# ucsdarclab/Python-SuPer

Measured on AMD Instinct MI355X. Metric: LM iterations/s (embedded-deformation LM, point-to-plane + ARAP + Rot), higher is better.
Workload: dtype f64; 1 GPU; C2: 200000 surfels / 2000 ED nodes / KNN=4, point-to-plane + ARAP + Rot, 10 LM iterations + Surfels.update per frame; frames_per_gpu=8, streams_per_gpu=1, global_frames=8, parallelism=frames sharded over 1 GPU(s), beta all-gather

## Files before the change

python-super_amd/csrc/slm_api.hip:

```cpp
#include <atomic>
#include <condition_variable>
#include <functional>
#include <mutex>
#include <new>
#include <string>
#include <thread>
#include <algorithm>
#include <vector>
#include <cstdio>
#include <cstring>

#include "slm_common.h"
#include "slm_corr.h"
#include "slm_host.h"
#include "slm_launch.h"
#include "slm_prep.h"

static thread_local std::string g_err;
static const char* const kBadKnn =
    "slm_bind_frame: a KNN index (sf_knn_idx or ed_knn_idx) lies outside [0, J) or a surfel's row of sf_knn_idx repeats an id";

void slm_set_error_text(const char* msg) { g_err = msg; }

namespace {
// ... 163 lines not shown

namespace {
class BindPool {
 public:
  ~BindPool() { shutdown(); }
  void run(int n, const std::function<void(int)>& job) {
    ensure(n - 1);
    {
      std::lock_guard<std::mutex> lk(m_);
      job_ = &job;
      n_active_ = n - 1;
      pending_ = n - 1;
      ++generation_;
    }
    cv_work_.notify_all();
    job(0);
    std::unique_lock<std::mutex> lk(m_);
    cv_done_.wait(lk, [&] { return pending_ == 0; });
    job_ = nullptr;
  }
  void shutdown() {
    {
      std::lock_guard<std::mutex> lk(m_);
      stop_ = true;
    }
    cv_work_.notify_all();
    for (std::thread& t : threads_)
      if (t.joinable()) t.join();
    threads_.clear();
  }

 private:
  void ensure(int n_workers) {
    while ((int)threads_.size() < n_workers) {
      const int id = (int)threads_.size();
      threads_.emplace_back([this, id] { loop(id); });
    }
  }
  void loop(int id) {
    int seen = 0;
    for (;;) {
      const std::function<void(int)>* job = nullptr;
      {
        std::unique_lock<std::mutex> lk(m_);
        cv_work_.wait(lk, [&] { return stop_ || generation_ != seen; });
        if (stop_) return;
        seen = generation_;
        if (id < n_active_) job = job_;
      }
      if (job) {
        (*job)(id + 1);
        std::lock_guard<std::mutex> lk(m_);
        if (--pending_ == 0) cv_done_.notify_all();
      }
    }
  }
  std::vector<std::thread> threads_;
  std::mutex m_;
  std::condition_variable cv_work_, cv_done_;
  const std::function<void(int)>* job_ = nullptr;
  int generation_ = 0, n_active_ = 0, pending_ = 0;
  bool stop_ = false;
};
}

struct slm_solver {
  PrepBuffers* prep = nullptr;
  BindPool bind_pool;
  AsyncWorker prep_worker;
  PrepBuffers* prep_async = nullptr;
  hipStream_t prep_stream = nullptr;
  std::vector<PrepBuffers*> bind_prep;
  std::vector<hipStream_t> bind_streams;
  std::vector<hipEvent_t> bind_events;
  std::mutex band_mutex;
  hipEvent_t drain_event = nullptr;
  double drain_est_ms = 0.0;
  int last_solver_form = -1;
  int last_dag_mode = -1;
  bool no_reuse = false;
  bool hybrid_batches = true;
  long dag_max_nodes = 8000;
  bool fuse_begin = true;
  bool pure_fill = true;
  bool profile = false;
  std::vector<hipEvent_t> ev_pool;
  std::vector<std::vector<hipEvent_t>> ev_runs;
  slm_config cfg{};
  std::vector<Slot> slots;
  FrameDev* frames_dev = nullptr;
  int* bw_dev = nullptr;
  int* bw_host = nullptr;
  int* reuse_dev = nullptr;
  int rank = 0, world = 1;
  int corr_mode = 0;
  double corr_w = 0.0;
  CorrDev* corr_dev = nullptr;
  bool shard_mode = false;
};
namespace {
bool solve_is_task_graph(const slm_solver* s, int n, int J);
}

static std::atomic<long long> g_reallocs{0}, g_realloc_bytes{0}, g_plan_builds{0}, g_plan_reuses{0}, g_plan_fill_hits{0};

template <typename T>
static hipError_t grow(T*& p, size_t& cap, size_t need) {
  if (need <= cap) return hipSuccess;
  const size_t want = need + need / 8;
  ++g_reallocs;
  g_realloc_bytes += (long long)(want * sizeof(T));
  return grow(p, cap, need, want);
}
template <typename T>
static hipError_t grow(GP<T>& p, size_t& cap, size_t need) {
  T* q = p;
  const hipError_t e = grow(q, cap, need);
  p = q;
  return e;
}

static int check_slots(slm_solver* s, int first, int n);

extern "C" {

const char* slm_last_error(void) { return g_err.c_str(); }

int slm_debug_last_solver_form(slm_solver* s) { return s ? s->last_solver_form : -1; }
int slm_debug_last_dag_mode(slm_solver* s) { return s ? s->last_dag_mode : -1; }

int slm_debug_counters(int64_t out[4]) {
  if (!out) return fail(SLM_ERR_INVALID, "slm_debug_counters: null output");
  out[0] = g_reallocs;
  out[1] = g_realloc_bytes;
  out[2] = g_plan_builds;
  out[3] = g_plan_reuses;
  return SLM_OK;
}

int slm_debug_dag_timeout(int64_t ticks) {
  if (ticks < 0) return fail(SLM_ERR_INVALID, "slm_debug_dag_timeout: negative");
  HIPCHK(set_dag_timeout_ticks(ticks == 0 ? 300000000ll : (long long)ticks));
  return SLM_OK;
}

int slm_debug_dag_abort(slm_solver* s, int32_t n_frames, void* stream) {
  int rc = check_slots(s, 0, n_frames);
  if (rc) return rc;
  for (int i = 0; i < n_frames; ++i)
    if (!s->slots[i].h.nd_ready) return fail(SLM_ERR_UNSUPPORTED, "slm_debug_dag_abort: every slot needs a nested-dissection plan");
  hipStream_t st = (hipStream_t)stream;
  launch_dag_abort_check(s->frames_dev, n_frames, st);
  launch_accept(s->frames_dev, n_frames, s->cfg.phase_test, 0, std::max(s->cfg.num_iterations, 1), st);
  HIPCHK(hipGetLastError());
  return SLM_OK;
}

int slm_debug_dag_trace(slm_solver* s, int32_t slot, int32_t on, void* stream) {
  if (!s || slot < 0 || slot >= (int)s->slots.size()) return fail(SLM_ERR_INVALID, "slm_debug_dag_trace: bad argument");
  Slot& sl = s->slots[slot];
  if (!sl.h.bound || !sl.h.nd_ready) return fail(SLM_ERR_UNBOUND, "slm_debug_dag_trace: no nested-dissection plan bound");
  hipStream_t st = (hipStream_t)stream;
  if (on) {
    HIPCHK(grow(sl.d_dag_trace, sl.cap_dag_trace, (size_t)24 * sl.h.n_dag_tasks + 8));
    HIPCHK(hipMemsetAsync(sl.d_dag_trace, 0, sizeof(long long) * 24 * (size_t)sl.h.n_dag_tasks, st));
  }
// ... 46 lines not shown
    case 4: src = h.blk_key.get(); n = sizeof(int32_t) * (size_t)h.n_blocks; break;
    case 5: src = h.blk_start.get(); n = sizeof(int32_t) * ((size_t)h.n_blocks + 1); break;
    case 6: src = h.blk_entry.get(); n = sizeof(int32_t) * 10 * (size_t)h.n_runs; break;
    case 7: src = h.v2_ready ? h.wg_first.get() : nullptr; n = h.v2_ready ? sizeof(int32_t) * n_wg : 0; break;
    case 8: src = h.v2_ready ? h.wg_last.get() : nullptr; n = h.v2_ready ? sizeof(int32_t) * n_wg : 0; break;
    case 9: src = h.v2_ready ? h.run_lidx.get() : nullptr; n = h.v2_ready ? 10 * (size_t)h.n_runs : 0; break;
    case 10: src = h.v2_ready ? h.blk2_start.get() : nullptr; n = h.v2_ready ? sizeof(int32_t) * ((size_t)h.n_blocks + 1) : 0; break;
    case 11: src = h.v2_ready ? h.blk2_entry.get() : nullptr; n = h.v2_ready ? sizeof(int32_t) * (size_t)h.n_wblk : 0; break;
    case 12: src = h.s_pts.get(); n = esz * 3 * (size_t)h.n_pos; break;
    default: return fail(SLM_ERR_INVALID, "slm_debug_read_plan: unknown array");
  }
  *n_bytes = (int64_t)n;
  const size_t m = n < (size_t)(max_bytes > 0 ? max_bytes : 0) ? n : (size_t)(max_bytes > 0 ? max_bytes : 0);
  if (m > 0 && host_out && src) HIPCHK(hipMemcpyAsync(host_out, src, m, hipMemcpyDeviceToHost, (hipStream_t)stream));
  HIPCHK(hipStreamSynchronize((hipStream_t)stream));
  return SLM_OK;
}

int slm_abi_version(void) { return SLM_ABI_VERSION; }

int slm_abi_check(int32_t abi_version, int32_t sz_config, int32_t sz_frame, int32_t sz_gf_config, int32_t sz_gf_frame,
                  int32_t sz_iter_record) {
  if (abi_version != SLM_ABI_VERSION || sz_config != (int32_t)sizeof(slm_config) || sz_frame != (int32_t)sizeof(slm_frame) ||
      sz_gf_config != (int32_t)sizeof(slm_gf_config) || sz_gf_frame != (int32_t)sizeof(slm_gf_frame) ||
      sz_iter_record != (int32_t)sizeof(slm_iter_record)) {
    char buf[320];
    snprintf(buf, sizeof(buf),
             "slm_abi_check: caller built for ABI %d (slm_config %d, slm_frame %d, slm_gf_config %d, slm_gf_frame %d, "
             "slm_iter_record %d bytes), library is ABI %d (%zu, %zu, %zu, %zu, %zu)",
             abi_version, sz_config, sz_frame, sz_gf_config, sz_gf_frame, sz_iter_record, SLM_ABI_VERSION, sizeof(slm_config),
             sizeof(slm_frame), sizeof(slm_gf_config), sizeof(slm_gf_frame), sizeof(slm_iter_record));
    return fail(SLM_ERR_INVALID, buf);
  }
  return SLM_OK;
}

int slm_device_count(void) {
  int n = 0;
  if (hipGetDeviceCount(&n) != hipSuccess) return 0;
  return n;
}

int slm_create(const slm_config* cfg, slm_solver** out) {
  if (!cfg || !out) return fail(SLM_ERR_INVALID, "slm_create: null argument");
  if (cfg->max_frames < 1 || cfg->num_iterations < 0 || !(cfg->v > 0.0))
    return fail(SLM_ERR_INVALID, "slm_create: bad config");
  if (cfg->solver_path < 0 || cfg->solver_path > 4) return fail(SLM_ERR_INVALID, "slm_create: solver_path must be 0..4");
  if (cfg->data_path < 0 || cfg->data_path > 2) return fail(SLM_ERR_INVALID, "slm_create: data_path must be 0..2");
  if (slm_device_count() < 1) return fail(SLM_ERR_NO_DEVICE, "slm_create: no HIP device visible");
  slm_solver* s = new (std::nothrow) slm_solver();
  if (!s) return fail(SLM_ERR_HIP, "slm_create: out of host memory");
  s->cfg = *cfg;
  try {
    s->slots.resize(cfg->max_frames);
  } catch (...) {
    delete s;
    return fail(SLM_ERR_HIP, "slm_create: out of host memory");
  }
  hipError_t e = hipMalloc((void**)&s->frames_dev, sizeof(FrameDev) * cfg->max_frames);
  if (e == hipSuccess) e = hipMemset(s->frames_dev, 0, sizeof(FrameDev) * cfg->max_frames);
  if (e == hipSuccess) e = hipMalloc((void**)&s->bw_dev, 2 * sizeof(int));
  if (e == hipSuccess) e = hipMalloc((void**)&s->reuse_dev, sizeof(int) * cfg->max_frames);
  if (e == hipSuccess) e = hipMemset(s->reuse_dev, 0, sizeof(int) * cfg->max_frames);
  if (e == hipSuccess) e = hipHostMalloc((void**)&s->bw_host, 2 * sizeof(int), hipHostMallocDefault);
  if (e == hipSuccess) {
    s->prep = prep_create();
    if (!s->prep) e = hipErrorOutOfMemory;
  }
  if (e != hipSuccess) {
    g_err = std::string("slm_create: ") + hipGetErrorString(e);
    slm_destroy(s);
    return SLM_ERR_HIP;
  }
  {
    int dev = 0;
    (void)hipGetDevice(&dev);
    (void)dag_device_setup(dev, nullptr);
  }
  if (const char* hb = getenv("SLM_HYBRID")) s->hybrid_batches = atoi(hb) != 0;
  if (const char* dm = getenv("SLM_DAG_MAX_NODES")) s->dag_max_nodes = atol(dm);
  if (const char* nr = getenv("SLM_NO_REUSE")) s->no_reuse = atoi(nr) != 0;
  if (const char* pf = getenv("SLM_PURE_FILL")) s->pure_fill = atoi(pf) != 0;
  if (const char* fb = getenv("SLM_FUSE_BEGIN")) s->fuse_begin = atoi(fb) != 0;
  *out = s;
  return SLM_OK;
}

int slm_destroy(slm_solver* s) {
  if (!s) return SLM_OK;
  s->prep_worker.shutdown();
  s->bind_pool.shutdown();
  for (Slot& sl : s->slots) {
    FrameDev& h = sl.h;
    if (h.beta) (void)hipFree(h.beta);
    if (h.delta) (void)hipFree(h.delta);
    if (h.rhs) (void)hipFree(h.rhs);
    if (sl.band) (void)hipFree(sl.band);
    if (sl.linv) (void)hipFree(sl.linv);
    if (h.loss_part) (void)hipFree(h.loss_part);
    if (h.st) (void)hipFree(h.st);
    if (h.rec) (void)hipFree(h.rec);
    if (h.node_pk) (void)hipFree(h.node_pk);
    if (h.tgt_pn) (void)hipFree(h.tgt_pn);
    if (h.tgt_px) (void)hipFree(h.tgt_px);
    if (h.ev_rc) (void)hipFree(h.ev_rc);
    plan_free(sl.plan);
    pairplan_free(sl.pplan);
    if (sl.h_pin) (void)hipHostFree(sl.h_pin);
    sl.h_pairs.release();
    sl.h_knn.release();
    sl.h_pts.release();
    sl.h_pts64.release();
    if (sl.d_fronts) (void)hipFree(sl.d_fronts);
    if (sl.d_items) (void)hipFree(sl.d_items);
    if (sl.d_tile_kind) (void)hipFree(sl.d_tile_kind);
    if (sl.d_zero_tiles) (void)hipFree(sl.d_zero_tiles);
    if (sl.d_ints) (void)hipFree(sl.d_ints);
    if (sl.d_dests) (void)hipFree(sl.d_dests);
    if (sl.d_cur_dests) (void)hipFree(sl.d_cur_dests);
    if (sl.ftiles) (void)hipFree(sl.ftiles);
    if (sl.fvec) (void)hipFree(sl.fvec);
    if (sl.flinv) (void)hipFree(sl.flinv);
    if (sl.fmail) (void)hipFree(sl.fmail);
    if (sl.pairbuf) (void)hipFree(sl.pairbuf);
    if (sl.corr.o) (void)hipFree(sl.corr.o);
    if (sl.corr.n) (void)hipFree(sl.corr.n);
    if (sl.corr.valid) (void)hipFree(sl.corr.valid);
    if (sl.d_dag_flags) (void)hipFree(sl.d_dag_flags);
    if (sl.d_dag_trace) (void)hipFree(sl.d_dag_trace);
    if (sl.prep_fork) (void)hipEventDestroy(sl.prep_fork);
    if (sl.prep_done) (void)hipEventDestroy(sl.prep_done);
  }
  prep_destroy(s->prep);
  prep_destroy(s->prep_async);
  if (s->prep_stream) (void)hipStreamDestroy(s->prep_stream);
  for (PrepBuffers* pb : s->bind_prep) prep_destroy(pb);
  for (hipStream_t q : s->bind_streams) (void)hipStreamDestroy(q);
  for (hipEvent_t e : s->bind_events) (void)hipEventDestroy(e);
  for (auto& evs : s->ev_runs)
    for (hipEvent_t e : evs)
      if (e) (void)hipEventDestroy(e);
  for (hipEvent_t e : s->ev_pool) (void)hipEventDestroy(e);
  if (s->drain_event) (void)hipEventDestroy(s->drain_event);
  if (s->frames_dev) (void)hipFree(s->frames_dev);
  if (s->bw_dev) (void)hipFree(s->bw_dev);
  if (s->reuse_dev) (void)hipFree(s->reuse_dev);
  if (s->corr_dev) (void)hipFree(s->corr_dev);
  if (s->bw_host) (void)hipHostFree(s->bw_host);
  delete s;
  return SLM_OK;
}

static int ensure_band(slm_solver* s, int slot, hipStream_t st) {
  Slot& sl = s->slots[slot];
  if (sl.band_ready) return SLM_OK;
  FrameDev& h = sl.h;
  launch_bandwidth(h.f, s->bw_dev, st);
  HIPCHK(hipMemcpyAsync(s->bw_host, s->bw_dev, 2 * sizeof(int), hipMemcpyDeviceToHost, st));
  HIPCHK(hipStreamSynchronize(st));
  if (s->bw_host[1]) return fail(SLM_ERR_INVALID, kBadKnn);
  int wb = *s->bw_host;
  if (wb > h.nt - 1) wb = h.nt - 1;
  h.wb = wb;
  HIPCHK(grow(sl.band, sl.cap_band, (size_t)h.nt * (wb + 1) * SLM_NB * SLM_NB));
  HIPCHK(grow(sl.linv, sl.cap_linv, (size_t)h.nt * SLM_NB * SLM_NB));
  h.band = sl.band;
// ... 669 lines not shown
  d.fused_begin = d.nd && tuple && d.gram_variants == 1 && d.max_pos > 0 && s->fuse_begin;
  if (tuple && c.phase_test) d.accept_reuse = s->reuse_dev + first;
  d.accept_eval = tuple ? 1 : 0;
  if (d.nd) {
    for (int i = first; i < first + n; ++i) {
      const auto& sc = s->slots[i].cache.nd.sched;
      if (sc.size() > d.sched.size()) d.sched.resize(sc.size(), NDLevelSched{0, 0, 0, 0, 0, -2, 0, -2, 0, -2});
      for (size_t l = 0; l < sc.size(); ++l) {
        NDLevelSched& m = d.sched[l];
        if (m.first == -2) m.first = sc[l].first;
        else if (m.first != sc[l].first || m.n_fronts != sc[l].n_fronts) m.first = -1;
        m.n_fronts = std::max(m.n_fronts, sc[l].n_fronts);
        m.max_npt = std::max(m.max_npt, sc[l].max_npt);
        m.max_nt = std::max(m.max_nt, sc[l].max_nt);
        m.max_pairs = std::max(m.max_pairs, sc[l].max_pairs);
        m.max_n2p = std::max(m.max_n2p, sc[l].max_n2p);
        if (m.schur_at == -2) m.schur_at = sc[l].schur_at;
        else if (m.schur_at != sc[l].schur_at || m.n_schur != sc[l].n_schur) m.schur_at = -1;
        m.n_schur = std::max(m.n_schur, sc[l].n_schur);
        if (m.pull_at == -2) m.pull_at = sc[l].pull_at;
        else if (m.pull_at != sc[l].pull_at || m.n_pull != sc[l].n_pull) m.pull_at = -1;
        m.n_pull = std::max(m.n_pull, sc[l].n_pull);
      }
    }
  }
  if (d.nd && n > 1) {
    for (int i = first; i < first + n; ++i)
      for (size_t l = s->slots[i].cache.nd.sched.size(); l < d.sched.size(); ++l)
        d.sched[l].first = d.sched[l].schur_at = d.sched[l].pull_at = -1;
  }
  for (auto& m : d.sched) {
    if (m.first == -2) m.first = -1;
    if (m.first < 0) m.schur_at = m.pull_at = -1;
    if (m.schur_at == -2) m.schur_at = -1;
    if (m.pull_at == -2) m.pull_at = -1;
  }
  if (s->cfg.use_arap || s->cfg.use_rot)
    d.n_reg_part = std::min(kRegBlocksMax, (d.maxJKe + 255) / 256);
  d.n_acc_part = d.n_reg_part + (s->corr_mode ? kCorrBlocks : 0);
  return d;
}

static bool solve_is_task_graph(const slm_solver* s, int n, int J) {
  return s->cfg.solver_path == 2 || (s->cfg.solver_path == 0 && (n <= 2 || (long)n * J <= s->dag_max_nodes));
}
static bool solve_is_hybrid(const slm_solver* s, int n, const BatchDims& d) {
  return !solve_is_task_graph(s, n, d.maxP / 7) && (s->cfg.solver_path == 4 || (s->cfg.solver_path == 0 && s->hybrid_batches)) &&
         d.hybrid_cut >= 0 && d.hybrid_levels == (int)d.sched.size() && d.hybrid_cut + 1 < d.hybrid_levels;
}
static int dag_cut_of(const slm_solver* s, int n, const BatchDims& d) {
  if (solve_is_task_graph(s, n, d.maxP / 7)) return -1;
  return solve_is_hybrid(s, n, d) ? d.hybrid_cut : -2;
}
int enqueue_front_solve(slm_solver* s, const FrameDev* fr, int n, const BatchDims& d, double u_override, hipStream_t st,
                        bool dag_reset_done = false, bool dag_check_later = false) {
  const bool dag = solve_is_task_graph(s, n, d.maxP / 7);
  const bool hybrid = solve_is_hybrid(s, n, d);
  s->last_solver_form = dag ? 1 : (hybrid ? 2 : 0);
  int mode = -1;
  if (dag) {
    mode = launch_front_solve_dag(fr, n, d.max_tasks, u_override, st, -1, !dag_reset_done, !dag_check_later);
  } else if (hybrid) {
    const int n_levels = (int)d.sched.size(), l_cut = n_levels - 1 - d.hybrid_cut;
    launch_front_levels(fr, n, d.sched.data(), n_levels, l_cut, 0, u_override, st);
    mode = launch_front_solve_dag(fr, n, d.max_top_tasks, u_override, st, d.hybrid_cut, !dag_reset_done, !dag_check_later);
  } else {
    launch_front_solve(fr, n, d.sched.data(), (int)d.sched.size(), u_override, st);
  }
  s->last_dag_mode = mode;
  return mode;
}

void enqueue_zero(const FrameDev* fr, int n, const BatchDims& d, hipStream_t st, const int* reuse, int dag_cut, bool fused) {
  if (!d.nd) launch_iter_begin(fr, n, st);
  else if (!fused) launch_iter_begin_nd(fr, n, st, reuse, dag_cut);
}

void enqueue_jacobian(slm_solver* s, const FrameDev* fr, int n, const BatchDims& d, hipStream_t st, int eval_mode,
                      const int* reuse, int dag_cut, bool fused) {
  const double w = s->cfg.w_data;
  switch (d.form) {
    case DataForm::tuple:
      if (eval_mode >= 0) launch_data_eval(fr, n, kLossBlocks, w, eval_mode, st, reuse);
      if (fused) launch_begin_and_gram(fr, n, d.max_pos, w, st, reuse, dag_cut);
      else launch_data_gram(fr, n, d.max_pos, w, d.gram_variants, st, reuse);
      break;
    case DataForm::pairs:
      launch_data_grad_pairs(fr, n, d.maxN, d.K, w, st);
      if (d.corr) launch_corr_grad_pairs(fr, s->corr_dev + (fr - s->frames_dev), n, d.maxN, d.K, s->corr_mode, s->corr_w, st);
      break;
    case DataForm::per_entry:
      launch_data_grad(fr, n, d.maxN, d.K, w, st);
      if (d.corr) launch_corr_grad(fr, s->corr_dev + (fr - s->frames_dev), n, d.maxN, d.K, s->corr_mode, s->corr_w, st);
      break;
    case DataForm::none: break;
  }
}

enum class Shard { whole, before_exchange, after_exchange };
void enqueue_scatter(slm_solver* s, const FrameDev* fr, int n, const BatchDims& d, hipStream_t st, Shard part) {
  const slm_config& c = s->cfg;
  const bool tuple = d.form == DataForm::tuple;
  if (part == Shard::before_exchange) {
    if (tuple) launch_pair_reduce(fr, n, d.max_blocks, st);
    return;
  }
  if (part == Shard::after_exchange || d.form == DataForm::pairs) launch_pair_scatter(fr, n, d.max_blocks, st);
  else if (tuple && d.nd) launch_front_assemble(fr, n, d.max_blocks, st);
  else if (tuple) launch_band_assemble(fr, n, d.max_blocks, st);
  if (d.nd) {
    launch_reg_grad_nd(fr, n, d.maxP / 7, c.use_arap, c.w_arap, c.use_rot, c.w_rot, st);
    if (!c.use_arap && !c.use_rot) launch_front_load_rhs(fr, n, d.maxP, st);
  } else {
    launch_reg_grad(fr, n, d.maxJKe, c.use_arap, c.w_arap, c.use_rot, c.w_rot, st);
  }
}

void enqueue_data_loss(slm_solver* s, const FrameDev* fr, int n, const BatchDims& d, hipStream_t st, bool at_beta) {
  if (d.form == DataForm::tuple && !at_beta) launch_data_eval(fr, n, kLossBlocks, s->cfg.w_data, 0, st);
  else if (d.form != DataForm::none) launch_data_loss(fr, n, kLossBlocks, d.K, s->cfg.w_data, at_beta ? 0 : 1, st);
  if (s->corr_mode && d.K >= 1)
    launch_corr_loss(fr, s->corr_dev + (fr - s->frames_dev), n, d.K, s->corr_mode, s->corr_w, at_beta ? 0 : 1, 2 * d.n_reg_part,
                     kCorrCntPart, st);
}
}

extern "C" {

static hipEvent_t take_event(slm_solver* s) {
  if (!s->ev_pool.empty()) {
    hipEvent_t e = s->ev_pool.back();
    s->ev_pool.pop_back();
    return e;
  }
  hipEvent_t e = nullptr;
  if (hipEventCreate(&e) != hipSuccess) return nullptr;
  return e;
}

int slm_set_shard(slm_solver* s, int32_t rank, int32_t world) {
  if (!s || world < 1 || rank < 0 || rank >= world) return fail(SLM_ERR_INVALID, "slm_set_shard: bad rank/world");
  if (s->cfg.data_path != 0 || s->cfg.solver_path == 1)
    return fail(SLM_ERR_UNSUPPORTED, "slm_set_shard: needs data_path 0 and a nested-dissection solver_path (0, 2, 3 or 4)");
  if (s->corr_mode)
    return fail(SLM_ERR_UNSUPPORTED, "slm_set_shard: the correspondence term is enabled (slm_enable_corr); it needs every surfel of "
                                     "the frame on one device");
  s->rank = rank;
  s->world = world;
  s->shard_mode = true;
  for (size_t i = 0; i < s->slots.size(); ++i) {
    join_prepare(s, (int)i);
    s->slots[i].model_ready = false;
    s->slots[i].h.bound = 0;
  }
  HIPCHK(hipMemset(s->frames_dev, 0, sizeof(FrameDev) * s->slots.size()));
  return SLM_OK;
}

static int shard_dims(slm_solver* s, int n_frames, BatchDims& d) {
  int rc = check_slots(s, 0, n_frames);
  if (rc) return rc;
  d = dims_of(s, 0, n_frames);
  if (!d.nd || (d.form != DataForm::tuple && d.form != DataForm::pairs))
    return fail(SLM_ERR_UNSUPPORTED, "sharded LM step: every slot needs a multifrontal data path (tuple-sorted or K-generic) and the ND solver");
  return SLM_OK;
}

int slm_lm_grad_local(slm_solver* s, int32_t n_frames, void* stream) {
// ... 582 lines not shown
```

python-super_amd/csrc/slm_begin.h:

```cpp
#pragma once
#include "slm_tile.h"

typedef double dvec2_t __attribute__((ext_vector_type(2)));
__device__ __forceinline__ void zero_pieces(double* base, size_t n_pieces, size_t first, size_t step) {
  const dvec2_t zz = {0.0, 0.0};
  dvec2_t* b2 = reinterpret_cast<dvec2_t*>(base);
  for (size_t pc = first; pc < n_pieces; pc += step) {
    dvec2_t* q = b2 + pc * 1024 + threadIdx.x;
#pragma unroll
    for (int k = 0; k < 4; ++k) __builtin_nontemporal_store(zz, q + 256 * k);
  }
}
__device__ __forceinline__ size_t front_piv_tiles(const NDFront& f) {
  return (size_t)f.npt * f.nt - (size_t)f.npt * (f.npt - 1) / 2;
}
__device__ __forceinline__ void zero_fronts(const FrameDev& fd, int b, int nb) {
  const dvec2_t zz = {0.0, 0.0};
  const int n = fd.n_zero_tiles;
  for (int pc = b; pc < 2 * n; pc += nb) {
    dvec2_t* q = reinterpret_cast<dvec2_t*>(fd.ftiles.get() + fd.zero_tiles[pc >> 1]) + (size_t)(pc & 1) * 1024 + threadIdx.x;
#pragma unroll
    for (int k = 0; k < 4; ++k) __builtin_nontemporal_store(zz, q + 256 * k);
  }
}
__device__ __forceinline__ void iter_begin_nd_body(const FrameDev& fd, int b, int nb, bool reused, int dag_cut, bool gram_sets_count) {
  if (!fd.bound) return;
  if (dag_cut >= -1 && fd.nd_ready && fd.dag_flags) {
    for (int i = b * blockDim.x + threadIdx.x; i < fd.dag_n_flags; i += nb * blockDim.x) fd.dag_flags[i] = 0;
    typedef __attribute__((address_space(1))) long long gll;
    gll* mail = (gll*)(double*)fd.fmail;
    for (int fi = b; fi < fd.n_fronts; fi += nb) {
      const NDFront& f = fd.fronts[fi];
      if (dag_cut >= 0 && f.depth > dag_cut) continue;
      const size_t base = (size_t)(f.linv_off / TILE) * SLM_MAIL_DOUBLES, n = (size_t)f.npt * SLM_MAIL_DOUBLES;
      for (size_t e = threadIdx.x; e < n; e += blockDim.x) mail[base + e] = SLM_MAIL_EMPTY;
    }
  }
  if (fd.st->stopped) return;
  const size_t tid = (size_t)b * blockDim.x + threadIdx.x, nthr = (size_t)nb * blockDim.x;
  const double2 z = make_double2(0.0, 0.0);
  if (fd.nd_ready) {
    zero_fronts(fd, b, nb);
    double2* v2 = reinterpret_cast<double2*>(fd.fvec.get());
    const size_t nv2 = (size_t)fd.zero_vec_doubles / 2;
    for (size_t e = tid; e < nv2; e += nthr) v2[e] = z;
  }
  const size_t nrhs = (size_t)fd.nt * SLM_NB;
  for (size_t e = tid; e < nrhs; e += nthr) fd.rhs[e] = 0.0;
  if (b == 0 && threadIdx.x == 0) {
    if (!reused) {
      if (!gram_sets_count) fd.st->m_grad = 0;
    } else if (fd.pairbuf) {
      fd.st->m_grad = fd.st->m_grad_local;
    }
    fd.st->chol_fail = 0;
  }
}
```

python-super_amd/csrc/slm_data_k4.hip:

```cpp
#include <cstdlib>

#include "slm_data.h"
#include "slm_begin.h"
#include "slm_launch.h"

#define ROW_STRIDE 17

__global__ void __launch_bounds__(256) k_data_eval(const FrameDev* __restrict__ frames, double lam, int mode,
                                                    const int* __restrict__ reuse) {
  __shared__ double sm[16];
  __shared__ int s_skip;
  if (mode == 1 && reuse && reuse[blockIdx.y]) return;
  const FrameDev& fd = frames[blockIdx.y];
  if (!fd.bound || !fd.v1_ready || fd.st->stopped) return;
  if (mode == 1) {
    if (threadIdx.x == 0) s_skip = __hip_atomic_load(&fd.st->eval_valid, __ATOMIC_RELAXED, __HIP_MEMORY_SCOPE_AGENT) == 1;
    __syncthreads();
    if (s_skip) return;
  }
  const double* npk = mode == 0 ? fd.node_pk_try.get() : fd.node_pk.get();
  const int p0 = 256 * fd.wg_lo, p1 = min(fd.n_pos, 256 * fd.wg_hi);
  double acc = 0.0;
  int cnt = 0;
  for (int pos = p0 + blockIdx.x * blockDim.x + threadIdx.x; pos < p1; pos += gridDim.x * blockDim.x) {
    const int4 ids = *reinterpret_cast<const int4*>(fd.s_idx + 4 * (size_t)pos);
    double2 o0 = make_double2(0.0, 0.0), o1 = make_double2(0.0, 0.0);
    if (ids.x >= 0) {
      double wk[4];
      ld_state4(fd.s_w, (size_t)pos, fd.f.state_f64, wk);
      const d3 pp = ld_state3(fd.s_pts, (size_t)pos, fd.f.state_f64);
      SurfelEval ev;
      eval_surfel_core<2, true>(fd, pp, ids, wk, lam, npk, ev);
      if (ev.match) {
        acc += ev.r * ev.r;
        ++cnt;
        o0 = make_double2(ev.r, ev.c[0]);
        o1 = make_double2(ev.c[1], ev.c[2]);
      }
    }
    double2* out = reinterpret_cast<double2*>(fd.ev_rc.get() + 4 * (size_t)pos);
    out[0] = o0;
    out[1] = o1;
  }
  const double s = block_sum(acc, sm);
  const double c = block_sum((double)cnt, sm);
  if (threadIdx.x == 0) {
    fd.loss_part[2 * blockIdx.x] = s;
    fd.loss_part[2 * blockIdx.x + 1] = c;
    LMState* st = fd.st;
    const unsigned long long old = __hip_atomic_fetch_add(&st->eval_acc, (1ull << 32) | (unsigned long long)(unsigned)(int)c,
                                                          __ATOMIC_RELAXED, __HIP_MEMORY_SCOPE_AGENT);
    if ((int)(old >> 32) == (int)gridDim.x - 1) {
      st->m_eval = (int)(unsigned)(old & 0xFFFFFFFFull) + (int)c;
      __hip_atomic_store(&st->eval_acc, 0ull, __ATOMIC_RELAXED, __HIP_MEMORY_SCOPE_AGENT);
      if (mode != 0) __hip_atomic_store(&st->eval_valid, 1, __ATOMIC_RELAXED, __HIP_MEMORY_SCOPE_AGENT);
    }
  }
}

template <bool MERGE, bool BEGIN = false>
__global__ void __launch_bounds__(256, 2) k_data_gram(const FrameDev* __restrict__ frames, double lam,
                                                       int dbg, const int* __restrict__ reuse, int n_gram = 0, int n_begin = 0,
                                                       int dag_cut = -2) {
  if (BEGIN && (int)blockIdx.x >= n_gram) {
    iter_begin_nd_body(frames[blockIdx.y], (int)blockIdx.x - n_gram, n_begin, reuse && reuse[blockIdx.y], dag_cut,
                       frames[blockIdx.y].v1_ready && frames[blockIdx.y].v2_ready);
    return;
  }
  __shared__ double rows[4][64 * ROW_STRIDE];
  __shared__ double recs[MERGE ? SLM_LB_MAX * SLM_WREC : 1];
  __shared__ uint8_t lidx[4][MERGE ? 160 : 4];
  if (reuse && reuse[blockIdx.y]) return;
  const FrameDev& fd = frames[blockIdx.y];
  if (!fd.bound || !fd.v1_ready) return;
  if (MERGE != (fd.v2_ready != 0)) return;
  const int w = threadIdx.x >> 6, l = threadIdx.x & 63;
  const int base = (blockIdx.x * 4 + w) * 64;
  if (blockIdx.x * 256 >= fd.n_pos) return;
  if (blockIdx.x == 0 && threadIdx.x == 0) fd.st->m_grad = fd.st->m_eval;
  if ((int)blockIdx.x < fd.wg_lo || (int)blockIdx.x >= fd.wg_hi) return;
  const bool wact = base < fd.n_pos;
  const int pos = base + l;
  const int lc = l & 15, lq = l >> 4;
  int rec0 = 0, nrec = 0;
  if (MERGE) {
    rec0 = fd.wg_first[blockIdx.x];
    nrec = fd.wg_last[blockIdx.x] - rec0 + 1;
  }
  int my_run = -1;
  int4 ids = {-1, -1, -1, -1};
  double wk[4] = {0, 0, 0, 0};
  d3 pp = {0, 0, 0};
  double2 e0 = make_double2(0.0, 0.0), e1 = make_double2(0.0, 0.0);
  if (wact) {
    my_run = fd.grp_run[(base >> 2) + lc];
    const double2* e2 = reinterpret_cast<const double2*>(fd.ev_rc.get() + 4 * (size_t)pos);
    e0 = e2[0];
    e1 = e2[1];
    ids = *reinterpret_cast<const int4*>(fd.s_idx + 4 * (size_t)pos);
    ld_state4(fd.s_w, (size_t)pos, fd.f.state_f64, wk);
    pp = ld_state3(fd.s_pts, (size_t)pos, fd.f.state_f64);
  }
  uint8_t lv0 = 0, lv1 = 0, lv2 = 0;
  if (MERGE && wact) {
#pragma unroll
    for (int k = 0; k < 3; ++k) {
      const int idx = l + 64 * k;
      const int g = idx / 10, e = idx - 10 * g;
      const int run = __shfl(my_run, g < 16 ? g : 0, 64);
      const uint8_t v = (idx < 160 && run >= 0) ? fd.run_lidx[10 * (size_t)run + e] : (uint8_t)0;
      if (k == 0) lv0 = v; else if (k == 1) lv1 = v; else lv2 = v;
    }
  }
  if (MERGE)
    for (int i = threadIdx.x; i < nrec * SLM_WREC; i += 256) recs[i] = 0.0;
  double* myrow = &rows[w][l * ROW_STRIDE];

  SurfelEval ev;
  ev.match = false;
  ev.r = 0.0;
  ev.id[0] = ev.id[1] = ev.id[2] = ev.id[3] = -1;
  const bool live = wact && ids.x >= 0;
#ifdef SLM_STAMPS
  if (live && !(dbg & 4))
#else
  if (live)
#endif
  {
    ev.id[0] = ids.x; ev.id[1] = ids.y; ev.id[2] = ids.z; ev.id[3] = ids.w;
    ev.match = e0.x != 0.0 || e0.y != 0.0 || e1.x != 0.0 || e1.y != 0.0;
    ev.r = e0.x;
    if (ev.match) rows_from_c(pp, ev.id, wk, lam, fd.node_pk, {e0.y, e1.x, e1.y}, ev.row);
  }
  if (MERGE && wact) {
    lidx[w][l] = lv0;
    lidx[w][l + 64] = lv1;
    if (l + 128 < 160) lidx[w][l + 128] = lv2;
  }
  if (MERGE) __syncthreads();
  if (wact) {

  int slot[4];
#pragma unroll
  for (int k = 0; k < 4; ++k) {
    slot[k] = 0;
#pragma unroll
    for (int k2 = 0; k2 < 4; ++k2) slot[k] += (ev.id[k2] < ev.id[k]) ? 1 : 0;
  }
  double a0[16];
#pragma unroll
  for (int half = 0; half < 2; ++half) {
#pragma unroll
    for (int e = 0; e < 16; ++e) myrow[e] = 0.0;
    if (ev.match) {
#pragma unroll
      for (int k = 0; k < 4; ++k)
#pragma unroll
        for (int c = 0; c < 7; ++c) {
          const int e = 7 * slot[k] + c - 16 * half;
          if (e >= 0 && e < 16) myrow[e] = ev.row[7 * k + c];
        }
      if (half == 1) myrow[28 - 16] = ev.r;
    }
    __builtin_amdgcn_fence(__ATOMIC_RELEASE, "wavefront");
    __builtin_amdgcn_wave_barrier();
    __builtin_amdgcn_fence(__ATOMIC_ACQUIRE, "wavefront");
    if (half == 0) {
#pragma unroll
      for (int g = 0; g < 16; ++g) a0[g] = rows[w][(4 * g + lq) * ROW_STRIDE + lc];
      __builtin_amdgcn_fence(__ATOMIC_RELEASE, "wavefront");
      __builtin_amdgcn_wave_barrier();
      __builtin_amdgcn_fence(__ATOMIC_ACQUIRE, "wavefront");
    }
  }

  double4_t g00 = {0, 0, 0, 0}, g10 = {0, 0, 0, 0}, g11 = {0, 0, 0, 0};
  int cur = -1;

  auto flush = [&](int run, int grp) {
#ifdef SLM_STAMPS
    if (dbg & 1) return;
#endif
    if (MERGE) {
      const uint8_t* lvp = &lidx[w][10 * grp];
#pragma unroll
      for (int t = 0; t < 3; ++t)
#pragma unroll
        for (int r = 0; r < 4; ++r) {
          const int i = 4 * r + lq + (t >= 1 ? 16 : 0), j = lc + (t == 2 ? 16 : 0);
          const double v = t == 0 ? g00[r] : (t == 1 ? g10[r] : g11[r]);
          const int pa = (i * 37) >> 8, pb = (j * 37) >> 8;
          const int ca = i - 7 * pa, cb = j - 7 * pb;
          const bool jrow = (i == 28);
          const bool act = j < 28 && (jrow || (i < 28 && i >= j));
          int ps = jrow ? (pb * (pb + 1) / 2 + pb) : (pa * (pa + 1) / 2 + pb);
          ps = act ? ps : 0;
          const int rec = lvp[ps];
          if (act) unsafeAtomicAdd(&recs[rec * SLM_WREC + (jrow ? 49 + cb : 7 * ca + cb)], v);
        }
    } else {
      double* out = fd.slab + (size_t)run * SLM_SLAB_STRIDE;
#pragma unroll
      for (int r = 0; r < 4; ++r) {
        out[r * 64 + l] = g00[r];
        out[256 + r * 64 + l] = g10[r];
        out[512 + r * 64 + l] = g11[r];
      }
    }
  };

#pragma unroll
  for (int g = 0; g < 16; ++g) {
    const int run = __builtin_amdgcn_readlane(my_run, g);
    if (run != cur) {
      if (cur >= 0) flush(cur, g - 1);
      g00 = double4_t{0, 0, 0, 0};
      g10 = double4_t{0, 0, 0, 0};
      g11 = double4_t{0, 0, 0, 0};
      cur = run;
    }
    if (run < 0) continue;
    const double a1 = rows[w][(4 * g + lq) * ROW_STRIDE + lc];
#ifdef SLM_STAMPS
    if (dbg & 2) { g00[0] += a0[g]; g11[0] += a1; continue; }
#endif
    g00 = __builtin_amdgcn_mfma_f64_16x16x4f64(a0[g], a0[g], g00, 0, 0, 0);
    g10 = __builtin_amdgcn_mfma_f64_16x16x4f64(a1, a0[g], g10, 0, 0, 0);
    g11 = __builtin_amdgcn_mfma_f64_16x16x4f64(a1, a1, g11, 0, 0, 0);
  }
  if (cur >= 0) flush(cur, 15);
  }
  if (MERGE) {
    __syncthreads();
    double* out = fd.wgslab + (size_t)rec0 * SLM_WREC;
    for (int i = threadIdx.x; i < nrec * SLM_WREC; i += 256) out[i] = recs[i];
  }
}

__device__ __forceinline__ double gram_at(const double* g, int i, int j) {
  if (i < 16) return g[16 * i + j];
  if (j < 16) return g[256 + 16 * (i - 16) + j];
  return g[512 + 16 * (i - 16) + (j - 16)];
}

__global__ void __launch_bounds__(256) k_band_assemble(const FrameDev* __restrict__ frames) {
  const FrameDev& fd = frames[blockIdx.y];
  if (!fd.bound || !fd.v1_ready || fd.st->stopped) return;
  const int bi = blockIdx.x * 4 + (threadIdx.x >> 6);
  if (bi >= fd.n_blocks) return;
  const int l = threadIdx.x & 63;
  const unsigned key = (unsigned)fd.blk_key[bi];
  const int a = (int)(key / (unsigned)fd.f.J), b = (int)(key % (unsigned)fd.f.J);
  const int ca = l / 7, cb = l % 7;
  const bool act = (l < 49) && (a != b || ca >= cb);
  const bool jt = (a == b) && l >= 49 && l < 56;
  double acc = 0.0;
  if (fd.v2_ready) {
    const int s0 = fd.blk2_start[bi], s1 = fd.blk2_start[bi + 1];
    if (l < SLM_WREC)
      for (int s = s0; s < s1; ++s) acc += fd.wgslab[(size_t)fd.blk2_entry[s] * SLM_WREC + l];
  } else {
    const int s0 = fd.blk_start[bi], s1 = fd.blk_start[bi + 1];
    for (int s = s0; s < s1; ++s) {
      const int pl = fd.blk_entry[s];
      const int run = pl >> 4, pa = (pl >> 2) & 3, pb = pl & 3;
      const double* G = fd.slab + (size_t)run * SLM_SLAB_STRIDE;
      if (act) acc += gram_at(G, 7 * pa + ca, 7 * pb + cb);
      else if (jt) acc += gram_at(G, 28, 7 * pa + (l - 49));
    }
  }
  if (act) *band_entry(fd, 7 * a + ca, 7 * b + cb) = acc;
  else if (jt) fd.rhs[7 * a + (l - 49)] = -acc;
}

void launch_begin_and_gram(const FrameDev* frames_dev, int n_frames, int max_pos, double lam, hipStream_t st, const int* reuse,
                           int dag_cut) {
  int dbg = 0;
#ifdef SLM_STAMPS
  if (const char* e = getenv("SLM_DBG")) dbg = atoi(e);
#endif
  const int n_gram = (max_pos + 255) / 256, n_begin = 1024;
  hipLaunchKernelGGL((k_data_gram<true, true>), dim3(n_gram + n_begin, n_frames), dim3(256), 0, st, frames_dev, lam, dbg, reuse, n_gram,
                     n_begin, dag_cut);
}

void launch_data_gram(const FrameDev* frames_dev, int n_frames, int max_pos, double lam, int variants,
                      hipStream_t st, const int* reuse) {
  if (max_pos <= 0) return;
  int dbg = 0;
#ifdef SLM_STAMPS
  if (const char* e = getenv("SLM_DBG")) dbg = atoi(e);
#endif
  const dim3 grid((max_pos + 255) / 256, n_frames);
  if (variants & 1) hipLaunchKernelGGL(k_data_gram<true>, grid, dim3(256), 0, st, frames_dev, lam, dbg, reuse);
  if (variants & 2) hipLaunchKernelGGL(k_data_gram<false>, grid, dim3(256), 0, st, frames_dev, lam, dbg, reuse);
}

void launch_data_eval(const FrameDev* frames_dev, int n_frames, int n_blocks, double lam, int mode, hipStream_t st,
                      const int* reuse) {
  hipLaunchKernelGGL(k_data_eval, dim3(n_blocks, n_frames), dim3(256), 0, st, frames_dev, lam, mode, reuse);
}

void launch_band_assemble(const FrameDev* frames_dev, int n_frames, int max_blocks, hipStream_t st) {
  if (max_blocks <= 0) return;
  hipLaunchKernelGGL(k_band_assemble, dim3((max_blocks + 3) / 4, n_frames), dim3(256), 0, st, frames_dev);
}
```

python-super_amd/csrc/slm_launch.h:

```cpp
#pragma once
#include "slm_common.h"

void launch_data_grad(const FrameDev*, int, int, int, double, hipStream_t);
void launch_data_grad_pairs(const FrameDev*, int, int, int, double, hipStream_t);
void launch_data_loss(const FrameDev*, int, int, int, double, int, hipStream_t);
void launch_data_resid(const FrameDev*, int, int, int, double, double*, uint8_t*, int32_t*, hipStream_t);

void launch_data_gram(const FrameDev*, int, int, double, int, hipStream_t, const int* reuse = nullptr);
void launch_begin_and_gram(const FrameDev*, int, int, double, hipStream_t, const int* reuse, int dag_cut);
void launch_data_eval(const FrameDev*, int, int, double, int mode, hipStream_t, const int* reuse = nullptr);
void launch_band_assemble(const FrameDev*, int, int, hipStream_t);

void launch_front_assemble(const FrameDev*, int, int, hipStream_t);
void launch_pair_reduce(const FrameDev*, int, int, hipStream_t);
void launch_pair_scatter(const FrameDev*, int, int, hipStream_t);
void launch_reg_grad_nd(const FrameDev*, int, int, int, double, int, double, hipStream_t);
void launch_front_load_rhs(const FrameDev*, int, int, hipStream_t);
void launch_iter_begin_nd(const FrameDev*, int, hipStream_t, const int* reuse, int dag_cut);
void launch_front_solve(const FrameDev*, int, const NDLevelSched*, int, double, hipStream_t);
void launch_front_levels(const FrameDev*, int, const NDLevelSched*, int, int, int, double, hipStream_t);

bool ensure_dynamic_lds(const void* kernel, size_t bytes);

int launch_front_solve_dag(const FrameDev*, int, int, double, hipStream_t, int cut, bool reset, bool check);
int dag_device_setup(int dev, int* xcd8_out);
int dag_last_mode();
hipError_t set_dag_timeout_ticks(long long);
void launch_dag_abort_check(const FrameDev*, int, hipStream_t);

void launch_bandwidth(const slm_frame&, int*, hipStream_t);
void launch_band_solve(const FrameDev*, int, int, int, double, hipStream_t);
void launch_band_to_dense(const FrameDev*, int, double*, hipStream_t);
void launch_dense_to_band(const FrameDev*, const double*, const double*, hipStream_t);

void launch_reg_grad(const FrameDev*, int, int, int, double, int, double, hipStream_t);
void launch_after_solve(const FrameDev*, int, int, int, int, double, int, double, int, hipStream_t);
void launch_reg_loss(const FrameDev*, int, int, int, double, int, double, int, hipStream_t);

void launch_init_slot(const FrameDev*, int, int, const slm_config&, hipStream_t);
void launch_iter_begin(const FrameDev*, int, hipStream_t);
void launch_pack_nodes(const FrameDev*, int, int, hipStream_t);
void launch_make_trial(const FrameDev*, int, int, hipStream_t);
void launch_pack_target(int, const float*, const float*, float4*, hipStream_t);
void launch_pack_target_px(int, const int*, const uint8_t*, const float*, const float*, float4*, hipStream_t);
void launch_accept(const FrameDev*, int, int, int, int, hipStream_t, int* reuse = nullptr, int eval_pass = 0);
void launch_loss_out(const FrameDev*, int, int, double*, hipStream_t);
void launch_zero_reg_part(const FrameDev*, int, int, hipStream_t);
void launch_update(int, int, int, float*, float*, const int*, const float*, float*, float*, const double*, hipStream_t);
void launch_update64(int, int, int, double*, double*, const int*, const double*, double*, double*, const double*,
                     hipStream_t);
void launch_knn(int, int, int, int, const float*, const float*, int*, float*, hipStream_t);
void launch_knn64(int, int, int, int, const double*, const double*, const int*, const int*, int*, double*, int*,
                  hipStream_t);
void launch_knn_weights64(int, int, int, const int*, const double*, const double*, int, const double*, const double*,
                          double*, uint8_t*, hipStream_t);
void launch_knn_weights(int, int, int, const int*, const float*, const float*, float*, uint8_t*, hipStream_t);
```

Before: 3335 LM it/s.

## Make data Gram kernel persistent with prefetch and interleaved front zeroing

Turns the k_data_gram kernel into a persistent grid sized from the CU count (2*CUs/frames by default, overridable by SLM_GRAM_WGS). Each workgroup loops over a contiguous range of 256-surfel chunks and software-prefetches the next chunk's inputs and lidx while computing the current one. In the fused begin variant, the front-tile zeroing that used to run in separate extra blocks is now spread across the same workgroups and interleaved with the chunk loop. The aim is to cut launch and tail overhead and to hide load latency behind MFMA work, at the cost of extra register pressure from the double-buffered chunk state and the risk of load imbalance across workgroups.

```diff
diff --git a/python-super_amd/csrc/slm_api.hip b/python-super_amd/csrc/slm_api.hip
--- a/python-super_amd/csrc/slm_api.hip
+++ b/python-super_amd/csrc/slm_api.hip
@@ -269,6 +269,8 @@
   bool hybrid_batches = true;
   long dag_max_nodes = 8000;
   bool fuse_begin = true;
+  int gram_wgs = 0;
+  int n_cus = 256;
   bool pure_fill = true;
   bool profile = false;
   std::vector<hipEvent_t> ev_pool;
@@ -481,6 +483,12 @@
   if (const char* nr = getenv("SLM_NO_REUSE")) s->no_reuse = atoi(nr) != 0;
   if (const char* pf = getenv("SLM_PURE_FILL")) s->pure_fill = atoi(pf) != 0;
   if (const char* fb = getenv("SLM_FUSE_BEGIN")) s->fuse_begin = atoi(fb) != 0;
+  if (const char* gw = getenv("SLM_GRAM_WGS")) s->gram_wgs = std::min(std::max(atoi(gw), 0), 65535);
+  {
+    int dev = 0, cus = 0;
+    (void)hipGetDevice(&dev);
+    if (hipDeviceGetAttribute(&cus, hipDeviceAttributeMultiprocessorCount, dev) == hipSuccess && cus > 0) s->n_cus = cus;
+  }
   *out = s;
   return SLM_OK;
 }
@@ -1316,8 +1324,8 @@
   switch (d.form) {
     case DataForm::tuple:
       if (eval_mode >= 0) launch_data_eval(fr, n, kLossBlocks, w, eval_mode, st, reuse);
-      if (fused) launch_begin_and_gram(fr, n, d.max_pos, w, st, reuse, dag_cut);
-      else launch_data_gram(fr, n, d.max_pos, w, d.gram_variants, st, reuse);
+      if (fused) launch_begin_and_gram(fr, n, w, st, reuse, dag_cut, s->gram_wgs, s->n_cus);
+      else launch_data_gram(fr, n, d.max_pos, w, d.gram_variants, st, reuse, s->gram_wgs, s->n_cus);
       break;
     case DataForm::pairs:
       launch_data_grad_pairs(fr, n, d.maxN, d.K, w, st);
diff --git a/python-super_amd/csrc/slm_begin.h b/python-super_amd/csrc/slm_begin.h
--- a/python-super_amd/csrc/slm_begin.h
+++ b/python-super_amd/csrc/slm_begin.h
@@ -23,7 +23,7 @@
     for (int k = 0; k < 4; ++k) __builtin_nontemporal_store(zz, q + 256 * k);
   }
 }
-__device__ __forceinline__ void iter_begin_nd_body(const FrameDev& fd, int b, int nb, bool reused, int dag_cut, bool gram_sets_count) {
+__device__ __forceinline__ void iter_begin_nd_small(const FrameDev& fd, int b, int nb, bool reused, int dag_cut, bool gram_sets_count) {
   if (!fd.bound) return;
   if (dag_cut >= -1 && fd.nd_ready && fd.dag_flags) {
     for (int i = b * blockDim.x + threadIdx.x; i < fd.dag_n_flags; i += nb * blockDim.x) fd.dag_flags[i] = 0;
@@ -40,7 +40,6 @@
   const size_t tid = (size_t)b * blockDim.x + threadIdx.x, nthr = (size_t)nb * blockDim.x;
   const double2 z = make_double2(0.0, 0.0);
   if (fd.nd_ready) {
-    zero_fronts(fd, b, nb);
     double2* v2 = reinterpret_cast<double2*>(fd.fvec.get());
     const size_t nv2 = (size_t)fd.zero_vec_doubles / 2;
     for (size_t e = tid; e < nv2; e += nthr) v2[e] = z;
@@ -56,3 +55,7 @@
     fd.st->chol_fail = 0;
   }
 }
+__device__ __forceinline__ void iter_begin_nd_body(const FrameDev& fd, int b, int nb, bool reused, int dag_cut, bool gram_sets_count) {
+  iter_begin_nd_small(fd, b, nb, reused, dag_cut, gram_sets_count);
+  if (fd.bound && fd.nd_ready && !fd.st->stopped) zero_fronts(fd, b, nb);
+}
diff --git a/python-super_amd/csrc/slm_data_k4.hip b/python-super_amd/csrc/slm_data_k4.hip
--- a/python-super_amd/csrc/slm_data_k4.hip
+++ b/python-super_amd/csrc/slm_data_k4.hip
@@ -58,87 +58,152 @@
   }
 }
 
+struct GramChunk {
+  int my_run;
+  int rec0, nrec;
+  int4 ids;
+  double2 e0, e1;
+  double2 wa, wb;
+  double px, py, pz;
+  float4 wf;
+  float qx, qy, qz;
+};
+template <bool MERGE>
+__device__ __forceinline__ void gram_chunk_load(const FrameDev& fd, int c, int w, int l, int f64, GramChunk& k) {
+  k.my_run = -1;
+  k.rec0 = k.nrec = 0;
+  k.ids = int4{-1, -1, -1, -1};
+  k.e0 = k.e1 = k.wa = k.wb = make_double2(0.0, 0.0);
+  k.px = k.py = k.pz = 0.0;
+  k.wf = make_float4(0.f, 0.f, 0.f, 0.f);
+  k.qx = k.qy = k.qz = 0.f;
+  if (MERGE) {
+    k.rec0 = fd.wg_first[c];
+    k.nrec = fd.wg_last[c] - k.rec0 + 1;
+  }
+  const int base = (c * 4 + w) * 64;
+  if (base >= fd.n_pos) return;
+  const size_t pos = (size_t)(base + l);
+  k.my_run = fd.grp_run[(base >> 2) + (l & 15)];
+  const double2* e2 = reinterpret_cast<const double2*>(fd.ev_rc.get() + 4 * pos);
+  k.e0 = e2[0];
+  k.e1 = e2[1];
+  k.ids = *reinterpret_cast<const int4*>(fd.s_idx + 4 * pos);
+  if (f64) {
+    const double2* q = reinterpret_cast<const double2*>(static_cast<const double*>(fd.s_w.get()) + 4 * pos);
+    k.wa = q[0];
+    k.wb = q[1];
+    const double* pq = static_cast<const double*>(fd.s_pts.get()) + 3 * pos;
+    k.px = pq[0]; k.py = pq[1]; k.pz = pq[2];
+  } else {
+    k.wf = *reinterpret_cast<const float4*>(static_cast<const float*>(fd.s_w.get()) + 4 * pos);
+    const float* pq = static_cast<const float*>(fd.s_pts.get()) + 3 * pos;
+    k.qx = pq[0]; k.qy = pq[1]; k.qz = pq[2];
+  }
+}
+__device__ __forceinline__ void gram_lidx_load(const FrameDev& fd, int my_run, int l, uint8_t lv[3]) {
+#pragma unroll
+  for (int k = 0; k < 3; ++k) {
+    const int idx = l + 64 * k;
+    const int g = idx / 10, e = idx - 10 * g;
+    const int run = __shfl(my_run, g < 16 ? g : 0, 64);
+    lv[k] = (idx < 160 && run >= 0) ? fd.run_lidx[10 * (size_t)run + e] : (uint8_t)0;
+  }
+}
+__device__ __forceinline__ void zero_front_piece(const FrameDev& fd, long long off, int pc) {
+  const dvec2_t zz = {0.0, 0.0};
+  dvec2_t* q = reinterpret_cast<dvec2_t*>(fd.ftiles.get() + off) + (size_t)(pc & 1) * 1024 + threadIdx.x;
+#pragma unroll
+  for (int k = 0; k < 4; ++k) __builtin_nontemporal_store(zz, q + 256 * k);
+}
+
 template <bool MERGE, bool BEGIN = false>
 __global__ void __launch_bounds__(256, 2) k_data_gram(const FrameDev* __restrict__ frames, double lam,
-                                                       int dbg, const int* __restrict__ reuse, int n_gram = 0, int n_begin = 0,
-                                                       int dag_cut = -2) {
-  if (BEGIN && (int)blockIdx.x >= n_gram) {
-    iter_begin_nd_body(frames[blockIdx.y], (int)blockIdx.x - n_gram, n_begin, reuse && reuse[blockIdx.y], dag_cut,
-                       frames[blockIdx.y].v1_ready && frames[blockIdx.y].v2_ready);
-    return;
-  }
+                                                       int dbg, const int* __restrict__ reuse, int dag_cut = -2) {
   __shared__ double rows[4][64 * ROW_STRIDE];
   __shared__ double recs[MERGE ? SLM_LB_MAX * SLM_WREC : 1];
   __shared__ uint8_t lidx[4][MERGE ? 160 : 4];
-  if (reuse && reuse[blockIdx.y]) return;
+  const bool reused = reuse && reuse[blockIdx.y];
+  if (!BEGIN && reused) return;
   const FrameDev& fd = frames[blockIdx.y];
-  if (!fd.bound || !fd.v1_ready) return;
-  if (MERGE != (fd.v2_ready != 0)) return;
+  const int b = blockIdx.x, nwg = gridDim.x;
   const int w = threadIdx.x >> 6, l = threadIdx.x & 63;
-  const int base = (blockIdx.x * 4 + w) * 64;
-  if (blockIdx.x * 256 >= fd.n_pos) return;
-  if (blockIdx.x == 0 && threadIdx.x == 0) fd.st->m_grad = fd.st->m_eval;
-  if ((int)blockIdx.x < fd.wg_lo || (int)blockIdx.x >= fd.wg_hi) return;
-  const bool wact = base < fd.n_pos;
-  const int pos = base + l;
   const int lc = l & 15, lq = l >> 4;
-  int rec0 = 0, nrec = 0;
-  if (MERGE) {
-    rec0 = fd.wg_first[blockIdx.x];
-    nrec = fd.wg_last[blockIdx.x] - rec0 + 1;
-  }
-  int my_run = -1;
-  int4 ids = {-1, -1, -1, -1};
-  double wk[4] = {0, 0, 0, 0};
-  d3 pp = {0, 0, 0};
-  double2 e0 = make_double2(0.0, 0.0), e1 = make_double2(0.0, 0.0);
-  if (wact) {
-    my_run = fd.grp_run[(base >> 2) + lc];
-    const double2* e2 = reinterpret_cast<const double2*>(fd.ev_rc.get() + 4 * (size_t)pos);
-    e0 = e2[0];
-    e1 = e2[1];
-    ids = *reinterpret_cast<const int4*>(fd.s_idx + 4 * (size_t)pos);
-    ld_state4(fd.s_w, (size_t)pos, fd.f.state_f64, wk);
-    pp = ld_state3(fd.s_pts, (size_t)pos, fd.f.state_f64);
-  }
-  uint8_t lv0 = 0, lv1 = 0, lv2 = 0;
-  if (MERGE && wact) {
-#pragma unroll
-    for (int k = 0; k < 3; ++k) {
-      const int idx = l + 64 * k;
-      const int g = idx / 10, e = idx - 10 * g;
-      const int run = __shfl(my_run, g < 16 ? g : 0, 64);
-      const uint8_t v = (idx < 160 && run >= 0) ? fd.run_lidx[10 * (size_t)run + e] : (uint8_t)0;
-      if (k == 0) lv0 = v; else if (k == 1) lv1 = v; else lv2 = v;
-    }
-  }
-  if (MERGE)
-    for (int i = threadIdx.x; i < nrec * SLM_WREC; i += 256) recs[i] = 0.0;
+  const int f64 = fd.f.state_f64;
+  int c0 = 0, c1 = 0;
+  if (!reused && fd.bound && fd.v1_ready && MERGE == (fd.v2_ready != 0) && fd.n_pos > 0) {
+    if (b == 0 && threadIdx.x == 0) fd.st->m_grad = fd.st->m_eval;
+    const int lo = max(fd.wg_lo, 0), hi = min(fd.wg_hi, (fd.n_pos + 255) >> 8);
+    if (hi > lo) {
+      c0 = lo + (int)((long long)(hi - lo) * b / nwg);
+      c1 = lo + (int)((long long)(hi - lo) * (b + 1) / nwg);
+    }
+  }
+  GramChunk cur{}, nxt{};
+  if (c0 < c1) gram_chunk_load<MERGE>(fd, c0, w, l, f64, cur);
+  int zk = 0, znv = 0, zper = 0;
+  if (BEGIN) {
+    iter_begin_nd_small(fd, b, nwg, reused, dag_cut, fd.v1_ready && fd.v2_ready);
+    if (fd.bound && fd.nd_ready && !fd.st->stopped) {
+      const int np = 2 * fd.n_zero_tiles;
+      znv = b < np ? (np - b + nwg - 1) / nwg : 0;
+      zper = c1 > c0 ? min(64, (znv + (c1 - c0) - 1) / (c1 - c0)) : 0;
+    }
+  }
+  if (MERGE && c0 < c1)
+    for (int i = threadIdx.x; i < SLM_LB_MAX * SLM_WREC; i += 256) recs[i] = 0.0;
   double* myrow = &rows[w][l * ROW_STRIDE];
-
-  SurfelEval ev;
-  ev.match = false;
-  ev.r = 0.0;
-  ev.id[0] = ev.id[1] = ev.id[2] = ev.id[3] = -1;
-  const bool live = wact && ids.x >= 0;
-#ifdef SLM_STAMPS
-  if (live && !(dbg & 4))
+  uint8_t lv[3] = {0, 0, 0};
+  if (MERGE && c0 < c1) gram_lidx_load(fd, cur.my_run, l, lv);
+
+  for (int c = c0; c < c1; ++c) {
+    const bool wact = (c * 4 + w) * 64 < fd.n_pos;
+    int znow = 0;
+    long long zoff = 0;
+    if (BEGIN) {
+      znow = min(zper, znv - zk);
+      if (l < znow) zoff = fd.zero_tiles[(b + (zk + l) * nwg) >> 1];
+    }
+    SurfelEval ev;
+    ev.match = false;
+    ev.r = 0.0;
+    ev.id[0] = ev.id[1] = ev.id[2] = ev.id[3] = -1;
+    const bool live = wact && cur.ids.x >= 0;
+#ifdef SLM_STAMPS
+    if (live && !(dbg & 4))
 #else
-  if (live)
-#endif
-  {
-    ev.id[0] = ids.x; ev.id[1] = ids.y; ev.id[2] = ids.z; ev.id[3] = ids.w;
-    ev.match = e0.x != 0.0 || e0.y != 0.0 || e1.x != 0.0 || e1.y != 0.0;
-    ev.r = e0.x;
-    if (ev.match) rows_from_c(pp, ev.id, wk, lam, fd.node_pk, {e0.y, e1.x, e1.y}, ev.row);
-  }
-  if (MERGE && wact) {
-    lidx[w][l] = lv0;
-    lidx[w][l + 64] = lv1;
-    if (l + 128 < 160) lidx[w][l + 128] = lv2;
-  }
-  if (MERGE) __syncthreads();
-  if (wact) {
+    if (live)
+#endif
+    {
+      ev.id[0] = cur.ids.x; ev.id[1] = cur.ids.y; ev.id[2] = cur.ids.z; ev.id[3] = cur.ids.w;
+      ev.match = cur.e0.x != 0.0 || cur.e0.y != 0.0 || cur.e1.x != 0.0 || cur.e1.y != 0.0;
+      ev.r = cur.e0.x;
+      if (ev.match) {
+        double wk[4];
+        d3 pp;
+        if (f64) {
+          wk[0] = cur.wa.x; wk[1] = cur.wa.y; wk[2] = cur.wb.x; wk[3] = cur.wb.y;
+          pp = {cur.px, cur.py, cur.pz};
+        } else {
+          wk[0] = (double)cur.wf.x; wk[1] = (double)cur.wf.y; wk[2] = (double)cur.wf.z; wk[3] = (double)cur.wf.w;
+          pp = {(double)cur.qx, (double)cur.qy, (double)cur.qz};
+        }
+        rows_from_c(pp, ev.id, wk, lam, fd.node_pk, {cur.e0.y, cur.e1.x, cur.e1.y}, ev.row);
+      }
+    }
+    const int my_run = cur.my_run, rec0 = cur.rec0, nrec = cur.nrec;
+    if (c + 1 < c1) gram_chunk_load<MERGE>(fd, c + 1, w, l, f64, nxt);
+    if (BEGIN) {
+      for (int k = 0; k < znow; ++k) zero_front_piece(fd, __shfl(zoff, k, 64), b + (zk + k) * nwg);
+      zk += znow;
+    }
+    if (MERGE && wact) {
+      lidx[w][l] = lv[0];
+      lidx[w][l + 64] = lv[1];
+      if (l + 128 < 160) lidx[w][l + 128] = lv[2];
+    }
+    if (MERGE) __syncthreads();
+    if (wact) {
 
   int slot[4];
 #pragma unroll
@@ -156,9 +221,9 @@
 #pragma unroll
       for (int k = 0; k < 4; ++k)
 #pragma unroll
-        for (int c = 0; c < 7; ++c) {
-          const int e = 7 * slot[k] + c - 16 * half;
-          if (e >= 0 && e < 16) myrow[e] = ev.row[7 * k + c];
+        for (int cc = 0; cc < 7; ++cc) {
+          const int e = 7 * slot[k] + cc - 16 * half;
+          if (e >= 0 && e < 16) myrow[e] = ev.row[7 * k + cc];
         }
       if (half == 1) myrow[28 - 16] = ev.r;
     }
@@ -175,7 +240,7 @@
   }
 
   double4_t g00 = {0, 0, 0, 0}, g10 = {0, 0, 0, 0}, g11 = {0, 0, 0, 0};
-  int cur = -1;
+  int crun = -1;
 
   auto flush = [&](int run, int grp) {
 #ifdef SLM_STAMPS
@@ -212,12 +277,12 @@
 #pragma unroll
   for (int g = 0; g < 16; ++g) {
     const int run = __builtin_amdgcn_readlane(my_run, g);
-    if (run != cur) {
-      if (cur >= 0) flush(cur, g - 1);
+    if (run != crun) {
+      if (crun >= 0) flush(crun, g - 1);
       g00 = double4_t{0, 0, 0, 0};
       g10 = double4_t{0, 0, 0, 0};
       g11 = double4_t{0, 0, 0, 0};
-      cur = run;
+      crun = run;
     }
     if (run < 0) continue;
     const double a1 = rows[w][(4 * g + lq) * ROW_STRIDE + lc];
@@ -228,13 +293,26 @@
     g10 = __builtin_amdgcn_mfma_f64_16x16x4f64(a1, a0[g], g10, 0, 0, 0);
     g11 = __builtin_amdgcn_mfma_f64_16x16x4f64(a1, a1, g11, 0, 0, 0);
   }
-  if (cur >= 0) flush(cur, 15);
-  }
-  if (MERGE) {
-    __syncthreads();
-    double* out = fd.wgslab + (size_t)rec0 * SLM_WREC;
-    for (int i = threadIdx.x; i < nrec * SLM_WREC; i += 256) out[i] = recs[i];
-  }
+  if (crun >= 0) flush(crun, 15);
+    }
+    if (MERGE) {
+      if (c + 1 < c1) gram_lidx_load(fd, nxt.my_run, l, lv);
+      __syncthreads();
+      double* out = fd.wgslab + (size_t)rec0 * SLM_WREC;
+      for (int i = threadIdx.x; i < nrec * SLM_WREC; i += 256) {
+        out[i] = recs[i];
+        recs[i] = 0.0;
+      }
+    }
+    cur = nxt;
+  }
+  if (BEGIN)
+    while (zk < znv) {
+      const int znow = min(64, znv - zk);
+      const long long zoff = l < znow ? fd.zero_tiles[(b + (zk + l) * nwg) >> 1] : 0;
+      for (int k = 0; k < znow; ++k) zero_front_piece(fd, __shfl(zoff, k, 64), b + (zk + k) * nwg);
+      zk += znow;
+    }
 }
 
 __device__ __forceinline__ double gram_at(const double* g, int i, int j) {
@@ -273,27 +351,28 @@
   else if (jt) fd.rhs[7 * a + (l - 49)] = -acc;
 }
 
-void launch_begin_and_gram(const FrameDev* frames_dev, int n_frames, int max_pos, double lam, hipStream_t st, const int* reuse,
-                           int dag_cut) {
+static int gram_wgs(int wgs, int n_frames, int n_cus) { return wgs > 0 ? wgs : max(1, 2 * n_cus / max(1, n_frames)); }
+
+void launch_begin_and_gram(const FrameDev* frames_dev, int n_frames, double lam, hipStream_t st, const int* reuse,
+                           int dag_cut, int wgs, int n_cus) {
   int dbg = 0;
 #ifdef SLM_STAMPS
   if (const char* e = getenv("SLM_DBG")) dbg = atoi(e);
 #endif
-  const int n_gram = (max_pos + 255) / 256, n_begin = 1024;
-  hipLaunchKernelGGL((k_data_gram<true, true>), dim3(n_gram + n_begin, n_frames), dim3(256), 0, st, frames_dev, lam, dbg, reuse, n_gram,
-                     n_begin, dag_cut);
+  hipLaunchKernelGGL((k_data_gram<true, true>), dim3(gram_wgs(wgs, n_frames, n_cus), n_frames), dim3(256), 0, st, frames_dev, lam, dbg,
+                     reuse, dag_cut);
 }
 
 void launch_data_gram(const FrameDev* frames_dev, int n_frames, int max_pos, double lam, int variants,
-                      hipStream_t st, const int* reuse) {
+                      hipStream_t st, const int* reuse, int wgs, int n_cus) {
   if (max_pos <= 0) return;
   int dbg = 0;
 #ifdef SLM_STAMPS
   if (const char* e = getenv("SLM_DBG")) dbg = atoi(e);
 #endif
-  const dim3 grid((max_pos + 255) / 256, n_frames);
-  if (variants & 1) hipLaunchKernelGGL(k_data_gram<true>, grid, dim3(256), 0, st, frames_dev, lam, dbg, reuse);
-  if (variants & 2) hipLaunchKernelGGL(k_data_gram<false>, grid, dim3(256), 0, st, frames_dev, lam, dbg, reuse);
+  const dim3 grid(wgs > 0 ? wgs : min(gram_wgs(0, n_frames, n_cus), (max_pos + 255) / 256), n_frames);
+  if (variants & 1) hipLaunchKernelGGL(k_data_gram<true>, grid, dim3(256), 0, st, frames_dev, lam, dbg, reuse, -2);
+  if (variants & 2) hipLaunchKernelGGL(k_data_gram<false>, grid, dim3(256), 0, st, frames_dev, lam, dbg, reuse, -2);
 }
 
 void launch_data_eval(const FrameDev* frames_dev, int n_frames, int n_blocks, double lam, int mode, hipStream_t st,
diff --git a/python-super_amd/csrc/slm_launch.h b/python-super_amd/csrc/slm_launch.h
--- a/python-super_amd/csrc/slm_launch.h
+++ b/python-super_amd/csrc/slm_launch.h
@@ -6,8 +6,8 @@
 void launch_data_loss(const FrameDev*, int, int, int, double, int, hipStream_t);
 void launch_data_resid(const FrameDev*, int, int, int, double, double*, uint8_t*, int32_t*, hipStream_t);
 
-void launch_data_gram(const FrameDev*, int, int, double, int, hipStream_t, const int* reuse = nullptr);
-void launch_begin_and_gram(const FrameDev*, int, int, double, hipStream_t, const int* reuse, int dag_cut);
+void launch_data_gram(const FrameDev*, int, int, double, int, hipStream_t, const int* reuse, int wgs, int n_cus);
+void launch_begin_and_gram(const FrameDev*, int, double, hipStream_t, const int* reuse, int dag_cut, int wgs, int n_cus);
 void launch_data_eval(const FrameDev*, int, int, double, int mode, hipStream_t, const int* reuse = nullptr);
 void launch_band_assemble(const FrameDev*, int, int, hipStream_t);
 
```

Result: faster. 3381 LM it/s, median of 6 (+1.4%).
